# Mikubill/sketch2img

Hardware: AMD Instinct MI355X
Metric: sketch-guided images/sec whole-node, SD1.5 512px 50-step DDIM (higher is better)
Workload: dtype fp16

## Files before the change

### sketch2img_amd/csrc/attention.hip

```cpp
#include "common.h"
#include <stdlib.h>
#include <type_traits>

namespace {

struct AttnParams {
  const half_t* Q; int ldq;
  const half_t* K; int ldk;
  const half_t* V; int ldv;
  const half_t* Vt; int ldvt;
  const half_t* dO; int lddo;
  half_t* O; int ldo;
  half_t* O2; int ldo2;
  float* lse;
  const float* delta;
  const half_t* Of; int ldof;
  float* delta_out;
  int batch, heads, Nq, Nkv, kv_stride, dh;
  float scale;
  int nx;
};

struct BlkMap { int bx, h, b; };
__device__ __forceinline__ BlkMap attn_block_map(const AttnParams& p) {
// ... 630 lines not shown
    soff[j] = ok ? (unsigned)(row * (isv ? p.ldvt : p.ldk) + pc * 8) * 2u : ATT_OOB;
    sdst[j] = ok ? (isv ? vrow * VP + pc * 8 : row * KP + pc * 8) : -1;
  }
  half8_t sreg[MAXPC], sreg2[DEEP ? MAXPC : 1];
  auto stage_load_to = [&](half8_t (&r)[MAXPC], int t) {
    const unsigned sk = (unsigned)t * 64u * (unsigned)p.ldk * 2u, sv = (unsigned)t * 64u * (unsigned)p.ldvt * 2u;
#pragma unroll
    for (int j = 0; j < MAXPC; ++j) r[j] = sisv[j] ? buf_half8(rv, soff[j], sv) : buf_half8(rk, soff[j], sk);
  };
  auto stage_store_from = [&](const half8_t (&r)[MAXPC], int t) {
    half_t* const ks = lds + (t & (NK - 1)) * KSZ;
    half_t* const vs = lds + VBASE + (t & (NV - 1)) * VSZ;
#pragma unroll
    for (int j = 0; j < MAXPC; ++j)
      if (sdst[j] >= 0) st_half8((sisv[j] ? vs : ks) + sdst[j], r[j]);
  };
  auto stage_load = [&](int t) { stage_load_to(sreg, t); };
  auto stage_store = [&](int t) { stage_store_from(sreg, t); };
  for (int i = tid; i < (NK + NV) * 64; i += NTHR) {
    const int slot = i >> 6, row = i & 63;
    if (slot < NK) {
      for (int c = PK * 8; c < D16 * 16; c += 8) st_half8(lds + slot * KSZ + row * KP + c, zero_half8());
    } else {
      half_t* const vr = lds + VBASE + (slot - NK) * VSZ + row * VP;
      if (ONES) {
        const half8_t one = {(half_t)1.f, 0, 0, 0, 0, 0, 0, 0};
        st_half8(vr + PK * 8, one);
      } else {
        for (int c = PK * 8; c < ND * 16; c += 8) st_half8(vr + c, zero_half8());
      }
    }
  }
  const int nt = (p.Nkv + 63) >> 6;
  stage_load(0);
  stage_store(0);
  if (nt > 1) { stage_load(1); stage_store(1); }
  if (nt > 2) stage_load(2);

  float16_t sA[2], sB[2];
  uint4_t pA[2][2], pB[2][2];
  float4_t o[2][ND];
  float nm = 0.f, l = 0.f;
#pragma unroll
  for (int qt = 0; qt < 2; ++qt)
#pragma unroll
    for (int u = 0; u < ND; ++u) o[qt][u] = float4_t{0.f, 0.f, 0.f, 0.f};
  constexpr float REF_SLACK = 8.f;
  const int vlane = (16 * (g >> 1) + 4 * (g & 1) + (l16 >> 2)) * VP + 4 * (l16 & 3);
  const int klane = l32 * KP + 8 * hi;

  auto read_k = [&](int t, half8_t (&kf)[2][D16]) {
    const half_t* Ks = lds + (t & (NK - 1)) * KSZ + klane;
#pragma unroll
    for (int kt = 0; kt < 2; ++kt)
#pragma unroll
      for (int ks = 0; ks < D16; ++ks) kf[kt][ks] = (PROBE & 16) ? qf[ks] : ld_half8(Ks + 32 * kt * KP + 16 * ks);
  };
  auto read_v = [&](int t, half8_t (&vf)[ND][2]) {
    const half_t* Vs = lds + VBASE + (t & (NV - 1)) * VSZ + vlane;
#pragma unroll
    for (int u = 0; u < ND; ++u)
#pragma unroll
      for (int sv = 0; sv < 2; ++sv) {
        if (PROBE & 16) { vf[u][sv] = qf[(u + sv) % D16]; continue; }
        const half4_t lo = tr_read(Vs + (32 * sv) * VP + 16 * u), hh = tr_read(Vs + (32 * sv + 8) * VP + 16 * u);
        vf[u][sv] = half8_t{lo[0], lo[1], lo[2], lo[3], hh[0], hh[1], hh[2], hh[3]};
      }
  };
  auto qk = [&](const half8_t (&kf)[2][D16], float16_t (&s)[2]) {
    if (PROBE & 2) { asm volatile("" : "+v"(s[0]), "+v"(s[1])); return; }
    const float16_t init = {nm, nm, nm, nm, nm, nm, nm, nm, nm, nm, nm, nm, nm, nm, nm, nm};
#pragma unroll
    for (int ks = 0; ks < D16; ++ks)
#pragma unroll
      for (int kt = 0; kt < 2; ++kt)
        s[kt] = __builtin_amdgcn_mfma_f32_32x32x16_f16(kf[kt][ks], qf[ks], ks == 0 ? init : s[kt], 0, 0, 0);
  };
  auto pv = [&](const half8_t (&vf)[ND][2], const uint4_t (&pb)[2][2]) {
    if (PROBE & 2) return;
#pragma unroll
    for (int sv = 0; sv < 2; ++sv)
#pragma unroll
      for (int u = 0; u < ND; ++u)
#pragma unroll
        for (int qt = 0; qt < 2; ++qt)
          o[qt][u] = __builtin_amdgcn_mfma_f32_16x16x32_f16(vf[u][sv], __builtin_bit_cast(half8_t, pb[qt][sv]), o[qt][u], 0, 0, 0);
  };
  auto expo = [&](const float16_t (&s)[2], uint4_t (&pb)[2][2]) {
    float ps = 0.f;
#pragma unroll
    for (int kt = 0; kt < 2; ++kt) {
      unsigned pk[8];
#pragma unroll
      for (int j = 0; j < 8; ++j) {
        const float e0 = (PROBE & 1) ? s[kt][2 * j] : __builtin_amdgcn_exp2f(s[kt][2 * j]);
        const float e1 = (PROBE & 1) ? s[kt][2 * j + 1] : __builtin_amdgcn_exp2f(s[kt][2 * j + 1]);
        if (!ONES) ps += e0 + e1;
        const half2_t h2 = {(half_t)e0, (half_t)e1};
        pk[j] = __builtin_bit_cast(unsigned, h2);
      }
#pragma unroll
      for (int j = 0; j < 4; ++j) {
        const auto r = __builtin_amdgcn_permlane16_swap(pk[j], pk[j + 4], false, false);
        pb[0][kt][j] = r[0];
        pb[1][kt][j] = r[1];
      }
    }
    if (!ONES) l += ps;
  };
  auto tile_max = [&](auto is_last, int t, float16_t (&s)[2]) {
    const int kv0 = t * 64;
    if (decltype(is_last)::value && kv0 + 64 > p.Nkv) {
      int lim = p.Nkv - kv0 - 4 * hi;
      asm volatile("" : "+v"(lim));
#pragma unroll
      for (int kt = 0; kt < 2; ++kt)
#pragma unroll
        for (int r = 0; r < 16; ++r)
          if (32 * kt + (r & 3) + 8 * (r >> 2) >= lim) s[kt][r] = NEG_BIG;
    }
    float m8[8];
#pragma unroll
    for (int j = 0; j < 5; ++j) m8[j] = max3f(s[0][3 * j], s[0][3 * j + 1], s[0][3 * j + 2]);
    m8[5] = max3f(s[0][15], s[1][0], s[1][1]);
    m8[6] = max3f(s[1][2], s[1][3], s[1][4]);
    m8[7] = max3f(s[1][5], s[1][6], s[1][7]);
    float mx = max3f(max3f(m8[0], m8[1], m8[2]), max3f(m8[3], m8[4], m8[5]), max3f(m8[6], m8[7], s[1][8]));
    mx = max3f(mx, max3f(s[1][9], s[1][10], s[1][11]), max3f(s[1][12], s[1][13], s[1][14]));
    return max3f(mx, s[1][15], mx);
  };
  auto rebase = [&](bool first, float mx, float16_t (&s)[2]) {
    mx = max3f(mx, __shfl_xor(mx, 32, 64), mx);
    const float delta = (first || mx > REF_SLACK) ? mx : 0.f;
    const float alpha = first ? 1.f : __builtin_amdgcn_exp2f(-delta);
    nm -= delta;
    l *= alpha;
    const float aA = __shfl(alpha, l16, 64), aB = __shfl(alpha, 16 + l16, 64);
#pragma unroll
    for (int u = 0; u < ND; ++u) { o[0][u] *= aA; o[1][u] *= aB; }
#pragma unroll
    for (int kt = 0; kt < 2; ++kt) s[kt] -= delta;
  };
#ifdef SKG_PHASES
  unsigned long long att_acc[6] = {0, 0, 0, 0, 0, 0};
#endif
  auto step = [&](auto has_pv, auto has_qk, int t, float16_t (&sc)[2], float16_t (&sn)[2], uint4_t (&pp)[2][2], uint4_t (&pc)[2][2]) {
    constexpr bool HAS_PV = decltype(has_pv)::value, HAS_QK = decltype(has_qk)::value;
    ATT_T(ta);
    half8_t vf[ND][2], kf[2][D16];
    if constexpr (HAS_PV) read_v(t - 1, vf);
    if constexpr (HAS_QK) read_k(t + 1, kf);
    if constexpr (HAS_PV) pv(vf, pp);
    const float mx = tile_max(std::integral_constant<bool, !HAS_QK>{}, t, sc);
    ATT_T(tb);
    if (__builtin_amdgcn_ballot_w64(t == 0 || mx > REF_SLACK) != 0) rebase(t == 0, mx, sc);
    ATT_T(tc);
    if constexpr (HAS_QK) qk(kf, sn);
    expo(sc, pc);
    ATT_T(td);
    if (!(PROBE & 4)) {
      if (t + 2 < nt) stage_store(t + 2);
      if (t + 3 < nt) stage_load(t + 3);
    }
    asm volatile("s_waitcnt lgkmcnt(0)" ::: "memory");
    ATT_T(te);
    __builtin_amdgcn_sched_barrier(0);
    if (!(PROBE & 8)) asm volatile("s_barrier" ::: "memory");
    __builtin_amdgcn_sched_barrier(0);
    ATT_T(tf);
    ATT_ACC(0, ta, tb); ATT_ACC(1, tb, tc); ATT_ACC(2, tc, td); ATT_ACC(3, td, te); ATT_ACC(4, te, tf); ATT_ACC(5, ta, tf);
  };
  using T_ = std::true_type;
  using F_ = std::false_type;
  if constexpr (DEEP) {
    half8_t kfA[2][D16], kfB[2][D16], vfA[ND][2], vfB[ND][2];
    auto dstep = [&](auto has_pv, auto has_qk, int t, float16_t (&sc)[2], float16_t (&sn)[2], uint4_t (&pp)[2][2], uint4_t (&pc)[2][2],
                     half8_t (&kfu)[2][D16], half8_t (&kff)[2][D16], half8_t (&vfu)[ND][2], half8_t (&vff)[ND][2], half8_t (&sst)[MAXPC]) {
      constexpr bool HAS_PV = decltype(has_pv)::value, HAS_QK = decltype(has_qk)::value;
      ATT_T(ta);
      if (t + 2 < nt) read_k(t + 2, kff);
      read_v(t, vff);
      if constexpr (HAS_PV) pv(vfu, pp);
      const float mx = tile_max(std::integral_constant<bool, !HAS_QK>{}, t, sc);
      ATT_T(tb);
      if (__builtin_amdgcn_ballot_w64(t == 0 || mx > REF_SLACK) != 0) rebase(t == 0, mx, sc);
      ATT_T(tc);
      if constexpr (HAS_QK) qk(kfu, sn);
      expo(sc, pc);
      ATT_T(td);
      if (!(PROBE & 4)) {
        if (t + 3 < nt) stage_store_from(sst, t + 3);
        if (t + 5 < nt) stage_load_to(sst, t + 5);
      }
      asm volatile("s_waitcnt lgkmcnt(0)" ::: "memory");
      ATT_T(te);
      __builtin_amdgcn_sched_barrier(0);
      if (!(PROBE & 8)) asm volatile("s_barrier" ::: "memory");
      __builtin_amdgcn_sched_barrier(0);
      ATT_T(tf);
      ATT_ACC(0, ta, tb); ATT_ACC(1, tb, tc); ATT_ACC(2, tc, td); ATT_ACC(3, td, te); ATT_ACC(4, te, tf); ATT_ACC(5, ta, tf);
    };
#define DSTEP_EVEN(PV_, QK_, t_) dstep(PV_{}, QK_{}, t_, sA, sB, pB, pA, kfB, kfA, vfB, vfA, sreg2)
#define DSTEP_ODD(PV_, QK_, t_) dstep(PV_{}, QK_{}, t_, sB, sA, pA, pB, kfA, kfB, vfA, vfB, sreg)
    __syncthreads();
    read_k(0, kfA);
    qk(kfA, sA);
    if (nt > 1) read_k(1, kfB);
    asm volatile("s_waitcnt lgkmcnt(0)\n\ts_barrier" ::: "memory");
    if (nt > 2) stage_store(2);
    if (nt > 3) stage_load_to(sreg2, 3);
    if (nt > 4) stage_load_to(sreg, 4);
    asm volatile("s_waitcnt lgkmcnt(0)\n\ts_barrier" ::: "memory");
    if (nt > 1) DSTEP_EVEN(F_, T_, 0); else DSTEP_EVEN(F_, F_, 0);
    int t = 1;
    for (; t + 2 < nt; t += 2) {
      DSTEP_ODD(T_, T_, t);
      DSTEP_EVEN(T_, T_, t + 1);
    }
    if (nt > 1) {
      if (t + 1 < nt) {
        DSTEP_ODD(T_, T_, t);
        DSTEP_EVEN(T_, F_, t + 1);
        pv(vfA, pA);
      } else {
        DSTEP_ODD(T_, F_, t);
        pv(vfB, pB);
      }
    } else {
      pv(vfA, pA);
    }
#undef DSTEP_EVEN
#undef DSTEP_ODD
  } else {

  __syncthreads();
  {
    half8_t kf[2][D16];
    read_k(0, kf);
    qk(kf, sA);
  }
  asm volatile("s_waitcnt lgkmcnt(0)\n\ts_barrier" ::: "memory");
  if (nt > 1) step(F_{}, T_{}, 0, sA, sB, pB, pA); else step(F_{}, F_{}, 0, sA, sB, pB, pA);
  int t = 1;
  for (; t + 2 < nt; t += 2) {
    step(T_{}, T_{}, t, sB, sA, pA, pB);
    step(T_{}, T_{}, t + 1, sA, sB, pB, pA);
  }
  bool last_in_a = true;
  if (nt > 1) {
    if (t + 1 < nt) {
      step(T_{}, T_{}, t, sB, sA, pA, pB);
      step(T_{}, F_{}, t + 1, sA, sB, pB, pA);
    } else {
      step(T_{}, F_{}, t, sB, sA, pA, pB);
      last_in_a = false;
    }
  }
  {
    half8_t vf[ND][2];
    read_v(nt - 1, vf);
    if (last_in_a) pv(vf, pA); else pv(vf, pB);
  }

  }
#ifdef SKG_PHASES
  if (lane == 0 && blockIdx.x < (1 << 13)) {
    for (int j = 0; j < 6; ++j) g_attn_phase[blockIdx.x * NW + wave][j] = att_acc[j];
    g_attn_phase[blockIdx.x * NW + wave][6] = nt;
  }
#endif
  float liA, liB;
  if (ONES) {
    liA = __shfl(o[0][ND - 1][0], 32 + l16, 64);
    liB = __shfl(o[1][ND - 1][0], 32 + l16, 64);
  } else {
    const float ls = l + __shfl_xor(l, 32, 64);
    liA = __shfl(ls, l16, 64);
    liB = __shfl(ls, 16 + l16, 64);
  }
#pragma unroll
  for (int qt = 0; qt < 2; ++qt) {
    const int q = q0 + 16 * qt + l16;
    const float inv = 1.f / (qt ? liB : liA);
    if (q < p.Nq) {
      half_t* orow = p.O + (size_t)(b * p.Nq + q) * p.ldo + h * dh;
#pragma unroll
      for (int u = 0; u < ND; ++u) {
        const int d = 16 * u + 4 * g;
        if (d < dh) {
          const half4_t v = {(half_t)(o[qt][u][0] * inv), (half_t)(o[qt][u][1] * inv), (half_t)(o[qt][u][2] * inv), (half_t)(o[qt][u][3] * inv)};
          st_half4(orow + d, v);
        }
      }
    }
  }
  if (p.lse) {
    const float li = (lane & 16) ? liB : liA;
    if (hi == 0 && q0 + l32 < p.Nq) p.lse[((size_t)b * p.heads + h) * p.Nq + q0 + l32] = (log2f(li) - nm) * LN2;
  }
}

#endif

template <int KS, int ND, int QT>
__global__ __launch_bounds__(256, 2) void attn_bwd_dq_kernel(const AttnParams p) {
  constexpr int KP = KS * 32 + 16;
  __shared__ __attribute__((aligned(16))) half_t Ks[64 * KP];
  __shared__ __attribute__((aligned(16))) half_t Vr[64 * KP];
  const int lane = threadIdx.x & 63, wave = threadIdx.x >> 6;
  const int l16 = lane & 15, g = lane >> 4;
  const BlkMap bm = attn_block_map(p);
  const int b = bm.b, h = bm.h;
  const int dh = p.dh;
  int q[QT];
  bool qok[QT];
  half8_t qf[QT][KS], dof[QT][KS];
  float4_t nlse[QT], ndl[QT];
  float4_t dq[QT][ND];
#pragma unroll
  for (int i = 0; i < QT; ++i) {
    q[i] = bm.bx * (64 * QT) + (wave * QT + i) * 16 + l16;
    qok[i] = q[i] < p.Nq;
#pragma unroll
    for (int ks = 0; ks < KS; ++ks) {
      const int c = 32 * ks + 8 * g;
      const bool ok = qok[i] && c < dh;
      qf[i][ks] = ok ? ld_half8(p.Q + (size_t)(b * p.Nq + q[i]) * p.ldq + h * dh + c) : zero_half8();
      dof[i][ks] = ok ? ld_half8(p.dO + (size_t)(b * p.Nq + q[i]) * p.lddo + h * dh + c) : zero_half8();
    }
    const size_t sidx = ((size_t)b * p.heads + h) * p.Nq + (qok[i] ? q[i] : 0);
    float dl;
    if (p.Of) {
      float sm = 0.f;
#pragma unroll
      for (int ks = 0; ks < KS; ++ks) {
        const int c = 32 * ks + 8 * g;
        if (qok[i] && c < dh) {
          const half8_t of = ld_half8(p.Of + (size_t)(b * p.Nq + q[i]) * p.ldof + h * dh + c);
#pragma unroll
          for (int j = 0; j < 8; ++j) sm += (float)of[j] * (float)dof[i][ks][j];
        }
      }
      sm += __shfl_xor(sm, 16, 64);
      sm += __shfl_xor(sm, 32, 64);
      if (g == 0 && qok[i]) p.delta_out[sidx] = sm;
      dl = sm;
    } else {
      dl = qok[i] ? p.delta[sidx] : 0.f;
    }
    const float nl = qok[i] ? -p.lse[sidx] * LOG2E : NEG_BIG, nd = qok[i] ? -dl : 0.f;
    nlse[i] = float4_t{nl, nl, nl, nl};
    ndl[i] = float4_t{nd, nd, nd, nd};
#pragma unroll
    for (int u = 0; u < ND; ++u) dq[i][u] = float4_t{0.f, 0.f, 0.f, 0.f};
  }
  const float sc = p.scale * LOG2E;
#pragma unroll
  for (int i = 0; i < QT; ++i)
#pragma unroll
    for (int ks = 0; ks < KS; ++ks)
#pragma unroll
      for (int j = 0; j < 8; ++j) qf[i][ks][j] = (half_t)((float)qf[i][ks][j] * sc);

  const half_t* Kb = p.K + (size_t)b * p.kv_stride * p.ldk + h * dh;
  const half_t* Vb = p.V + (size_t)b * p.kv_stride * p.ldv + h * dh;
  const int nt = (p.Nkv + 63) / 64;
  RowRegs<KS> rk, rv;
  const RowSrc<KS> sk = row_src<KS>(Kb, p.ldk, p.kv_stride, dh), sv = row_src<KS>(Vb, p.ldv, p.kv_stride, dh);
  const int tlane = (4 * g + (l16 >> 2)) * KP + 4 * (l16 & 3);
  rows_load_buf<KS>(rk, sk, p.ldk, 0);
  rows_load_buf<KS>(rv, sv, p.ldv, 0);
  for (int t0 = 0; t0 < nt; ++t0) {
    const int kv0 = t0 * 64;
    __syncthreads();
    rows_store<KS>(rk, Ks);
    rows_store<KS>(rv, Vr);
    __syncthreads();
    if (t0 + 1 < nt) {
      rows_load_buf<KS>(rk, sk, p.ldk, kv0 + 64);
      rows_load_buf<KS>(rv, sv, p.ldv, kv0 + 64);
    }
    float4_t s[QT][4], dp[QT][4];
#pragma unroll
    for (int t = 0; t < 4; ++t) {
#pragma unroll
      for (int ks = 0; ks < KS; ++ks) {
        const int off = (16 * t + l16) * KP + 32 * ks + 8 * g;
        const half8_t kfr = ld_half8(Ks + off), vfr = ld_half8(Vr + off);
#pragma unroll
        for (int i = 0; i < QT; ++i) {
          s[i][t] = __builtin_amdgcn_mfma_f32_16x16x32_f16(kfr, qf[i][ks], ks == 0 ? nlse[i] : s[i][t], 0, 0, 0);
          dp[i][t] = __builtin_amdgcn_mfma_f32_16x16x32_f16(vfr, dof[i][ks], ks == 0 ? ndl[i] : dp[i][t], 0, 0, 0);
        }
      }
    }
    half8_t sb[QT][2];
#pragma unroll
    for (int i = 0; i < QT; ++i) {
      if (kv0 + 64 > p.Nkv) {
        const int lim = p.Nkv - kv0 - 4 * g;
#pragma unroll
        for (int t = 0; t < 4; ++t)
#pragma unroll
          for (int r = 0; r < 4; ++r)
            if (16 * t + r >= lim) s[i][t][r] = NEG_BIG;
      }
#pragma unroll
      for (int t = 0; t < 4; ++t)
#pragma unroll
        for (int r = 0; r < 4; ++r) s[i][t][r] = __builtin_amdgcn_exp2f(s[i][t][r]) * dp[i][t][r];
      pack_p(s[i], sb[i]);
    }
#pragma unroll
    for (int u = 0; u < ND; ++u)
#pragma unroll
      for (int k2 = 0; k2 < 2; ++k2) {
        const half8_t ktf = tfrag_rows<KP>(Ks + tlane, u, k2);
#pragma unroll
        for (int i = 0; i < QT; ++i) dq[i][u] = __builtin_amdgcn_mfma_f32_16x16x32_f16(ktf, sb[i][k2], dq[i][u], 0, 0, 0);
      }
  }
#pragma unroll
  for (int i = 0; i < QT; ++i) {
    if (!qok[i]) continue;
    half_t* orow = p.O + (size_t)(b * p.Nq + q[i]) * p.ldo + h * dh;
#pragma unroll
    for (int u = 0; u < ND; ++u) {
      const int d = 16 * u + 4 * g;
      if (d < dh) {
        half4_t v = {(half_t)(dq[i][u][0] * p.scale), (half_t)(dq[i][u][1] * p.scale), (half_t)(dq[i][u][2] * p.scale),
                     (half_t)(dq[i][u][3] * p.scale)};
        st_half4(orow + d, v);
      }
    }
  }
}

template <int KS, int ND, int KT>
__global__ __launch_bounds__(256, (KS >= 5 ? 1 : 2)) void attn_bwd_dkv_kernel(const AttnParams p) {
  constexpr int KP = KS * 32 + 16;
  __shared__ __attribute__((aligned(16))) half_t Qs[64 * KP];
  __shared__ __attribute__((aligned(16))) half_t Ds[64 * KP];
  __shared__ __attribute__((aligned(16))) float lse_s[64], del_s[64];
  const int lane = threadIdx.x & 63, wave = threadIdx.x >> 6;
  const int l16 = lane & 15, g = lane >> 4;
  const BlkMap bm = attn_block_map(p);
  const int b = bm.b, h = bm.h;
  const int dh = p.dh;
  int kv[KT];
  bool kok[KT];
  half8_t kf[KT][KS], vf[KT][KS];
#pragma unroll
  for (int i = 0; i < KT; ++i) {
    kv[i] = bm.bx * (64 * KT) + (wave * KT + i) * 16 + l16;
    kok[i] = kv[i] < p.Nkv;
#pragma unroll
    for (int ks = 0; ks < KS; ++ks) {
      const int c = 32 * ks + 8 * g;
      const bool ok = kok[i] && c < dh;
      kf[i][ks] = ok ? ld_half8(p.K + (size_t)(b * p.kv_stride + kv[i]) * p.ldk + h * dh + c) : zero_half8();
      vf[i][ks] = ok ? ld_half8(p.V + (size_t)(b * p.kv_stride + kv[i]) * p.ldv + h * dh + c) : zero_half8();
    }
  }
  const float sc = p.scale * LOG2E;
#pragma unroll
  for (int i = 0; i < KT; ++i)
#pragma unroll
    for (int ks = 0; ks < KS; ++ks)
#pragma unroll
      for (int j = 0; j < 8; ++j) kf[i][ks][j] = (half_t)((float)kf[i][ks][j] * sc);
  float4_t dk[KT][ND], dv[KT][ND];
#pragma unroll
  for (int i = 0; i < KT; ++i)
#pragma unroll
    for (int u = 0; u < ND; ++u) {
      dk[i][u] = float4_t{0.f, 0.f, 0.f, 0.f};
      dv[i][u] = float4_t{0.f, 0.f, 0.f, 0.f};
    }
  const half_t* Qb = p.Q + (size_t)b * p.Nq * p.ldq + h * dh;
  const half_t* Db = p.dO + (size_t)b * p.Nq * p.lddo + h * dh;
  const size_t sbase = ((size_t)b * p.heads + h) * p.Nq;
  const int nt = (p.Nq + 63) / 64;
  RowRegs<KS> rq, rd;
  float r_lse = 0.f, r_del = 0.f;
  const RowSrc<KS> sq = row_src<KS>(Qb, p.ldq, p.Nq, dh), sd = row_src<KS>(Db, p.lddo, p.Nq, dh);
  const int tlane = (4 * g + (l16 >> 2)) * KP + 4 * (l16 & 3);
  auto prefetch = [&](int q0) {
    rows_load_buf<KS>(rq, sq, p.ldq, q0);
    rows_load_buf<KS>(rd, sd, p.lddo, q0);
    if (threadIdx.x < 64) {
      const int qq = q0 + threadIdx.x;
      r_lse = qq < p.Nq ? -p.lse[sbase + qq] * LOG2E : NEG_BIG;
      r_del = qq < p.Nq ? -p.delta[sbase + qq] : 0.f;
    }
  };
  prefetch(0);
  for (int t0 = 0; t0 < nt; ++t0) {
    const int q0 = t0 * 64;
    __syncthreads();
    rows_store<KS>(rq, Qs);
    rows_store<KS>(rd, Ds);
    if (threadIdx.x < 64) { lse_s[threadIdx.x] = r_lse; del_s[threadIdx.x] = r_del; }
    __syncthreads();
    if (t0 + 1 < nt) prefetch(q0 + 64);
    float4_t s[KT][4], dp[KT][4];
#pragma unroll
    for (int t = 0; t < 4; ++t) {
      const float4_t nl = *reinterpret_cast<const float4_t*>(lse_s + 16 * t + 4 * g);
#pragma unroll
      for (int ks = 0; ks < KS; ++ks) {
        const int off = (16 * t + l16) * KP + 32 * ks + 8 * g;
        const half8_t qfr = ld_half8(Qs + off), dfr = ld_half8(Ds + off);
#pragma unroll
        for (int i = 0; i < KT; ++i) {
          s[i][t] = __builtin_amdgcn_mfma_f32_16x16x32_f16(qfr, kf[i][ks], ks == 0 ? nl : s[i][t], 0, 0, 0);
          dp[i][t] = __builtin_amdgcn_mfma_f32_16x16x32_f16(dfr, vf[i][ks], ks == 0 ? float4_t{0.f, 0.f, 0.f, 0.f} : dp[i][t], 0, 0, 0);
        }
      }
    }
    half8_t pb[KT][2], sb[KT][2];
#pragma unroll
    for (int i = 0; i < KT; ++i) {
      float4_t ds[4];
#pragma unroll
      for (int t = 0; t < 4; ++t)
#pragma unroll
        for (int r = 0; r < 4; ++r) {
          const float pr = __builtin_amdgcn_exp2f(s[i][t][r]);
          s[i][t][r] = pr;
          ds[t][r] = pr * (dp[i][t][r] + del_s[16 * t + 4 * g + r]);
        }
      pack_p(s[i], pb[i]);
      pack_p(ds, sb[i]);
    }
#pragma unroll
    for (int u = 0; u < ND; ++u)
#pragma unroll
      for (int k2 = 0; k2 < 2; ++k2) {
        const half8_t dtf = tfrag_rows<KP>(Ds + tlane, u, k2), qtf = tfrag_rows<KP>(Qs + tlane, u, k2);
#pragma unroll
        for (int i = 0; i < KT; ++i) {
          dv[i][u] = __builtin_amdgcn_mfma_f32_16x16x32_f16(dtf, pb[i][k2], dv[i][u], 0, 0, 0);
          dk[i][u] = __builtin_amdgcn_mfma_f32_16x16x32_f16(qtf, sb[i][k2], dk[i][u], 0, 0, 0);
        }
      }
  }
#pragma unroll
  for (int i = 0; i < KT; ++i) {
    if (!kok[i]) continue;
    half_t* krow = p.O + (size_t)(b * p.kv_stride + kv[i]) * p.ldo + h * dh;
    half_t* vrow = p.O2 + (size_t)(b * p.kv_stride + kv[i]) * p.ldo2 + h * dh;
#pragma unroll
    for (int u = 0; u < ND; ++u) {
      const int d = 16 * u + 4 * g;
      if (d < dh) {
        half4_t a = {(half_t)(dk[i][u][0] * p.scale), (half_t)(dk[i][u][1] * p.scale),
                     (half_t)(dk[i][u][2] * p.scale), (half_t)(dk[i][u][3] * p.scale)};
        half4_t c = {(half_t)dv[i][u][0], (half_t)dv[i][u][1], (half_t)dv[i][u][2], (half_t)dv[i][u][3]};
        st_half4(krow + d, a);
        st_half4(vrow + d, c);
      }
    }
  }
}

__global__ __launch_bounds__(256) void attn_delta_kernel(const half_t* __restrict__ O, int ldo,
                                                         const half_t* __restrict__ dO, int lddo,
                                                         float* __restrict__ delta, int batch, int heads, int Nq,
                                                         int dh) {
  const size_t total = (size_t)batch * Nq * heads;
  const size_t item = ((size_t)blockIdx.x * 256 + threadIdx.x) >> 4;
  const int sub = threadIdx.x & 15;
  float s = 0.f;
  if (item < total) {
    const int h = (int)(item % heads);
    const size_t row = item / heads;
    for (int c = sub * 8; c < dh; c += 128) {
      const half8_t a = ld_half8(O + row * ldo + h * dh + c);
      const half8_t d = ld_half8(dO + row * lddo + h * dh + c);
#pragma unroll
      for (int j = 0; j < 8; ++j) s += (float)a[j] * (float)d[j];
    }
  }
#pragma unroll
  for (int o = 8; o > 0; o >>= 1) s += __shfl_xor(s, o, 64);
  if (item < total && sub == 0) {
    const int h = (int)(item % heads);
    const size_t row = item / heads;
    const size_t b = row / Nq, q = row - b * Nq;
    delta[(b * heads + h) * Nq + q] = s;
  }
}

inline int attn_var();
template <int KS, int ND, bool VROW>
static void attn_fwd_launch_qt(AttnParams& p, hipStream_t st) {
  const int var = attn_var();
  const long rows = (long)p.heads * p.batch;
  if constexpr (ND == 3) {
    if (var == 9 || (var == 0 && skg_cdiv(p.Nq, 192) * rows >= 1024)) {
      p.nx = skg_cdiv(p.Nq, 192);
      hipLaunchKernelGGL((attn_fwd_kernel<KS, ND, 3, false, 2 | (3 << 2), VROW>), dim3((unsigned)(p.nx * rows)), dim3(256), 0, st, p);
      return;
    }
  } else if constexpr (VROW) {
    if (var == 8) {
      p.nx = skg_cdiv(p.Nq, 256);
      hipLaunchKernelGGL((attn_fwd_kernel<KS, ND, 4, false, 2 | (2 << 2), VROW>), dim3((unsigned)(p.nx * rows)), dim3(256), 0, st, p);
      return;
    }
  }
  p.nx = skg_cdiv(p.Nq, 128);
  const dim3 grid((unsigned)(p.nx * rows));
  if (ND == 4 && var != 7)
    hipLaunchKernelGGL((attn_fwd_kernel<KS, ND, 2, false, 2 | (3 << 2), VROW>), grid, dim3(256), 0, st, p);
  else
    hipLaunchKernelGGL((attn_fwd_kernel<KS, ND, 2, false, 0, VROW>), grid, dim3(256), 0, st, p);
}
#define SKG_ATTN_VARIANTS(KS_, ND_, grid2, VROW_) attn_fwd_launch_qt<KS_, ND_, VROW_>(p, st)

#define SKG_ATTN_FWD_DISPATCH(grid1, grid2, VROW_)                                                                 \
  switch (p.dh) {                                                                                                  \
    case 16: hipLaunchKernelGGL((attn_fwd_kernel<1, 1, 2, false, 0, VROW_>), grid2, dim3(256), 0, st, p); break;   \
    case 32: hipLaunchKernelGGL((attn_fwd_kernel<1, 2, 2, false, 0, VROW_>), grid2, dim3(256), 0, st, p); break;   \
    case 40: SKG_ATTN_VARIANTS(2, 3, grid2, VROW_); break;                                                         \
    case 64: SKG_ATTN_VARIANTS(2, 4, grid2, VROW_); break;                                                         \
    case 80: hipLaunchKernelGGL((attn_fwd_kernel<3, 5, 2, false, 0, VROW_>), grid2, dim3(256), 0, st, p); break;   \
    case 160: hipLaunchKernelGGL((attn_fwd_kernel<5, 10, 1, false, 0, VROW_>), grid1, dim3(256), 0, st, p); break; \
    default: return SKG_E_UNSUPPORTED;                                                                             \
  }

#define SKG_ATTN_FWD_CAUSAL_DISPATCH(grid2)                                                               \
  switch (p.dh) {                                                                                        \
    case 16: hipLaunchKernelGGL((attn_fwd_kernel<1, 1, 2, true>), grid2, dim3(256), 0, st, p); break;    \
    case 32: hipLaunchKernelGGL((attn_fwd_kernel<1, 2, 2, true>), grid2, dim3(256), 0, st, p); break;    \
    case 64: hipLaunchKernelGGL((attn_fwd_kernel<2, 4, 2, true>), grid2, dim3(256), 0, st, p); break;    \
    default: return SKG_E_UNSUPPORTED;                                                                   \
  }

inline int attn_var() {
  static const int v = getenv("SKG_ATTN_VAR") ? atoi(getenv("SKG_ATTN_VAR")) : 0;
  return v;
}

inline bool common_ok(int batch, int heads, int Nq, int Nkv, int kv_stride, int dh, bool kv8 = true) {
  return batch > 0 && heads > 0 && Nq > 0 && Nkv > 0 && kv_stride >= Nkv && (!kv8 || kv_stride % 8 == 0) && dh % 8 == 0;
}

}

extern "C" int skg_attn_fwd(const void* Q, int ldq, const void* K, int ldk, const void* Vt, int ldvt, void* O,
                            int ldo, float* lse, int batch, int heads, int Nq, int Nkv, int kv_stride, int dh,
                            float scale, unsigned flags, void* stream) {
  const bool causal = flags & SKG_ATTN_CAUSAL, vrow = flags & SKG_ATTN_ROWV, resident = flags & SKG_ATTN_RESIDENT_KV;
  SKG_REQUIRE(!(flags & ~(SKG_ATTN_CAUSAL | SKG_ATTN_ROWV | SKG_ATTN_RESIDENT_KV)) && !(causal && vrow) && (!resident || vrow));
  SKG_REQUIRE(Q && K && Vt && O && common_ok(batch, heads, Nq, Nkv, kv_stride, dh, !vrow));
  SKG_REQUIRE(ldq % 8 == 0 && ldk % 8 == 0 && ldvt % 8 == 0 && ldo % 4 == 0);
  SKG_REQUIRE(skg_aligned(Q, 16) && skg_aligned(K, 16) && skg_aligned(Vt, 16) && skg_aligned(O, 8));
  AttnParams p{};
  p.Q = (const half_t*)Q; p.ldq = ldq; p.K = (const half_t*)K; p.ldk = ldk; p.Vt = (const half_t*)Vt; p.ldvt = ldvt;
  p.O = (half_t*)O; p.ldo = ldo; p.lse = lse;
  p.batch = batch; p.heads = heads; p.Nq = Nq; p.Nkv = Nkv; p.kv_stride = kv_stride; p.dh = dh; p.scale = scale;
  hipStream_t st = (hipStream_t)stream;
  static const bool no_short = getenv("SKG_NO_ATTN_SHORT") != nullptr;
  if (vrow && !causal && kv_stride <= 80 && !no_short && (dh == 40 || dh == 64 || dh == 80 || dh == 160)) {
    long qch = ((long)heads * batch * Nq / 1024 + 63) / 64 * 64;
    qch = qch < 64 ? 64 : (qch > 512 ? 512 : qch);
    p.nx = skg_cdiv(Nq, (int)qch);
    dim3 gs((unsigned)p.nx * heads * batch);
    switch (dh) {
      case 40: hipLaunchKernelGGL((attn_fwd_short_kernel<2, 3>), gs, dim3(256), 0, st, p, (int)qch); break;
      case 64: hipLaunchKernelGGL((attn_fwd_short_kernel<2, 4>), gs, dim3(256), 0, st, p, (int)qch); break;
      case 80: hipLaunchKernelGGL((attn_fwd_short_kernel<3, 5>), gs, dim3(256), 0, st, p, (int)qch); break;
      default: hipLaunchKernelGGL((attn_fwd_short_kernel<5, 10>), gs, dim3(256), 0, st, p, (int)qch); break;
    }
    SKG_CHECK_LAUNCH("skg_attn_fwd (short keys)");
    return SKG_OK;
  }
  const int rtiles = kv_stride <= 160 ? 10 : 15;
  if (resident && kv_stride > 80 && kv_stride <= 240 && !no_short && (dh == 40 || dh == 64 || dh == 80 || (dh == 160 && rtiles == 10))) {
    long qch = ((long)heads * batch * Nq / 1024 + 63) / 64 * 64;
    qch = qch < 128 ? 128 : (qch > 512 ? 512 : qch);
    p.nx = skg_cdiv(Nq, (int)qch);
    dim3 gs((unsigned)p.nx * heads * batch);
    if (rtiles == 10) {
      switch (dh) {
        case 40: hipLaunchKernelGGL((attn_fwd_short_kernel<2, 3, 10>), gs, dim3(256), 0, st, p, (int)qch); break;
        case 64: hipLaunchKernelGGL((attn_fwd_short_kernel<2, 4, 10>), gs, dim3(256), 0, st, p, (int)qch); break;
        case 80: hipLaunchKernelGGL((attn_fwd_short_kernel<3, 5, 10>), gs, dim3(256), 0, st, p, (int)qch); break;
        default: hipLaunchKernelGGL((attn_fwd_short_kernel<5, 10, 10>), gs, dim3(256), 0, st, p, (int)qch); break;
      }
    } else {
      switch (dh) {
        case 40: hipLaunchKernelGGL((attn_fwd_short_kernel<2, 3, 15>), gs, dim3(256), 0, st, p, (int)qch); break;
        case 64: hipLaunchKernelGGL((attn_fwd_short_kernel<2, 4, 15>), gs, dim3(256), 0, st, p, (int)qch); break;
        default: hipLaunchKernelGGL((attn_fwd_short_kernel<3, 5, 15>), gs, dim3(256), 0, st, p, (int)qch); break;
      }
    }
    SKG_CHECK_LAUNCH("skg_attn_fwd (resident keys)");
    return SKG_OK;
  }
#if defined(SKG_LAB) || defined(SKG_PHASES)
  static const bool no8 = getenv("SKG_NO_ATTN8") != nullptr || getenv("SKG_ATTN8") == nullptr;
  static const int form8 = getenv("SKG_ATTN8") ? atoi(getenv("SKG_ATTN8")) : 0;
  if (vrow && !causal && !no8 && (dh == 40 || dh == 64) && (long)skg_cdiv(Nq, 256) * heads * batch >= 192) {
    const int qpw = form8 == 2 ? 128 : 256;
    p.nx = skg_cdiv(Nq, qpw);
    dim3 g8((unsigned)p.nx * heads * batch);
#ifdef SKG_PHASES
    static const int probe8 = getenv("SKG_ATTN8_PROBE") ? atoi(getenv("SKG_ATTN8_PROBE")) : 0;
    if (probe8 && dh == 40 && form8 == 2) {
      switch (probe8) {
        case 1: hipLaunchKernelGGL((attn_fwd8_kernel<3, 3, true, 4, 3, 1>), g8, dim3(256), 0, st, p); break;
        case 2: hipLaunchKernelGGL((attn_fwd8_kernel<3, 3, true, 4, 3, 2>), g8, dim3(256), 0, st, p); break;
        case 4: hipLaunchKernelGGL((attn_fwd8_kernel<3, 3, true, 4, 3, 4>), g8, dim3(256), 0, st, p); break;
        case 8: hipLaunchKernelGGL((attn_fwd8_kernel<3, 3, true, 4, 3, 8>), g8, dim3(256), 0, st, p); break;
        case 12: hipLaunchKernelGGL((attn_fwd8_kernel<3, 3, true, 4, 3, 12>), g8, dim3(256), 0, st, p); break;
        case 16: hipLaunchKernelGGL((attn_fwd8_kernel<3, 3, true, 4, 3, 16>), g8, dim3(256), 0, st, p); break;
        case 28: hipLaunchKernelGGL((attn_fwd8_kernel<3, 3, true, 4, 3, 28>), g8, dim3(256), 0, st, p); break;
        case 29: hipLaunchKernelGGL((attn_fwd8_kernel<3, 3, true, 4, 3, 29>), g8, dim3(256), 0, st, p); break;
        default: hipLaunchKernelGGL((attn_fwd8_kernel<3, 3, true, 4, 3, 30>), g8, dim3(256), 0, st, p); break;
      }
      SKG_CHECK_LAUNCH("skg_attn_fwd (8 waves, probe)");
      return SKG_OK;
    }
#endif
    if (form8 == 2) {
      if (dh == 40) hipLaunchKernelGGL((attn_fwd8_kernel<3, 3, true, 4, 3>), g8, dim3(256), 0, st, p);
      else hipLaunchKernelGGL((attn_fwd8_kernel<4, 4, false, 4, 2>), g8, dim3(256), 0, st, p);
    } else {
      if (dh == 40) hipLaunchKernelGGL((attn_fwd8_kernel<3, 3, true>), g8, dim3(512), 0, st, p);
      else hipLaunchKernelGGL((attn_fwd8_kernel<4, 4, false>), g8, dim3(512), 0, st, p);
    }
    SKG_CHECK_LAUNCH("skg_attn_fwd (8 waves)");
    return SKG_OK;
  }
#endif
  p.nx = skg_cdiv(Nq, dh == 160 ? 64 : 128);
  dim3 grid((unsigned)p.nx * heads * batch);
  if (causal) {
    SKG_REQUIRE(dh != 160 && !vrow);
    SKG_ATTN_FWD_CAUSAL_DISPATCH(grid);
  } else if (vrow) {
    SKG_ATTN_FWD_DISPATCH(grid, grid, true);
  } else {
    SKG_ATTN_FWD_DISPATCH(grid, grid, false);
  }
  SKG_CHECK_LAUNCH("skg_attn_fwd");
  return SKG_OK;
}

extern "C" int skg_attn_bwd_delta(const void* O, int ldo, const void* dO, int lddo, float* delta, int batch,
                                  int heads, int Nq, int dh, void* stream) {
  SKG_REQUIRE(O && dO && delta && batch > 0 && heads > 0 && Nq > 0 && dh % 8 == 0 && ldo % 8 == 0 && lddo % 8 == 0);
  SKG_REQUIRE(skg_aligned(O, 16) && skg_aligned(dO, 16));
  const size_t total = (size_t)batch * Nq * heads;
  hipLaunchKernelGGL(attn_delta_kernel, dim3((unsigned)((total * 16 + 255) / 256)), dim3(256), 0,
                     (hipStream_t)stream, (const half_t*)O, ldo, (const half_t*)dO, lddo, delta, batch, heads, Nq, dh);
  SKG_CHECK_LAUNCH("skg_attn_bwd_delta");
  return SKG_OK;
}

extern "C" int skg_attn_bwd_dq(const void* Q, int ldq, const void* K, int ldk, const void* V, int ldv, const void* dO, int lddo,
                               const void* O, int ldo, const float* lse, const float* delta, float* delta_out, void* dQ, int lddq,
                               int batch, int heads, int Nq, int Nkv, int kv_stride, int dh, float scale, void* stream) {
  if (delta) { O = nullptr; ldo = 0; delta_out = nullptr; }
  SKG_REQUIRE(Q && K && V && dO && lse && (delta || (O && delta_out)) && dQ && common_ok(batch, heads, Nq, Nkv, kv_stride, dh, false));
  SKG_REQUIRE(!O || (ldo % 8 == 0 && skg_aligned(O, 16)));
  SKG_REQUIRE(ldq % 8 == 0 && ldk % 8 == 0 && ldv % 8 == 0 && lddo % 8 == 0 && lddq % 4 == 0);
  SKG_REQUIRE(skg_aligned(Q, 16) && skg_aligned(K, 16) && skg_aligned(V, 16) && skg_aligned(dO, 16) && skg_aligned(dQ, 8));
  AttnParams p{};
  p.Q = (const half_t*)Q; p.ldq = ldq; p.K = (const half_t*)K; p.ldk = ldk; p.V = (const half_t*)V; p.ldv = ldv;
  p.dO = (const half_t*)dO; p.lddo = lddo;
  p.lse = const_cast<float*>(lse); p.delta = delta; p.O = (half_t*)dQ; p.ldo = lddq;
  p.Of = (const half_t*)O; p.ldof = ldo; p.delta_out = delta_out;
  p.batch = batch; p.heads = heads; p.Nq = Nq; p.Nkv = Nkv; p.kv_stride = kv_stride; p.dh = dh; p.scale = scale;
  hipStream_t st = (hipStream_t)stream;
  p.nx = skg_cdiv(Nq, dh <= 40 ? 128 : 64);
  dim3 grid((unsigned)p.nx * heads * batch);
  switch (dh) {
    case 16: hipLaunchKernelGGL((attn_bwd_dq_kernel<1, 1, 2>), grid, dim3(256), 0, st, p); break;
    case 32: hipLaunchKernelGGL((attn_bwd_dq_kernel<1, 2, 2>), grid, dim3(256), 0, st, p); break;
    case 40: hipLaunchKernelGGL((attn_bwd_dq_kernel<2, 3, 2>), grid, dim3(256), 0, st, p); break;
    case 64: hipLaunchKernelGGL((attn_bwd_dq_kernel<2, 4, 1>), grid, dim3(256), 0, st, p); break;
    case 80: hipLaunchKernelGGL((attn_bwd_dq_kernel<3, 5, 1>), grid, dim3(256), 0, st, p); break;
    case 160: hipLaunchKernelGGL((attn_bwd_dq_kernel<5, 10, 1>), grid, dim3(256), 0, st, p); break;
    default: return SKG_E_UNSUPPORTED;
  }
  SKG_CHECK_LAUNCH("skg_attn_bwd_dq");
  return SKG_OK;
}

extern "C" int skg_attn_bwd_dkv(const void* Q, int ldq, const void* K, int ldk,
                                const void* V, int ldv, const void* dO, int lddo,
                                const float* lse, const float* delta, void* dK, int lddk, void* dV, int lddv,
                                int batch, int heads, int Nq, int Nkv, int kv_stride, int dh, float scale, void* stream) {
  SKG_REQUIRE(Q && K && V && dO && lse && delta && dK && dV && common_ok(batch, heads, Nq, Nkv, kv_stride, dh, false));
  SKG_REQUIRE(ldq % 8 == 0 && ldk % 8 == 0 && ldv % 8 == 0 && lddo % 8 == 0 && lddk % 4 == 0 && lddv % 4 == 0);
  SKG_REQUIRE(skg_aligned(Q, 16) && skg_aligned(K, 16) && skg_aligned(V, 16) &&
              skg_aligned(dO, 16) && skg_aligned(dK, 8) && skg_aligned(dV, 8));
  AttnParams p{};
  p.Q = (const half_t*)Q; p.ldq = ldq; p.K = (const half_t*)K; p.ldk = ldk;
  p.V = (const half_t*)V; p.ldv = ldv; p.dO = (const half_t*)dO; p.lddo = lddo;
  p.lse = const_cast<float*>(lse); p.delta = delta; p.O = (half_t*)dK; p.ldo = lddk;
  p.O2 = (half_t*)dV; p.ldo2 = lddv;
  p.batch = batch; p.heads = heads; p.Nq = Nq; p.Nkv = Nkv; p.kv_stride = kv_stride; p.dh = dh; p.scale = scale;
  hipStream_t st = (hipStream_t)stream;
  p.nx = skg_cdiv(Nkv, dh <= 40 ? 128 : 64);
  dim3 grid((unsigned)p.nx * heads * batch);
  switch (dh) {
    case 16: hipLaunchKernelGGL((attn_bwd_dkv_kernel<1, 1, 2>), grid, dim3(256), 0, st, p); break;
    case 32: hipLaunchKernelGGL((attn_bwd_dkv_kernel<1, 2, 2>), grid, dim3(256), 0, st, p); break;
    case 40: hipLaunchKernelGGL((attn_bwd_dkv_kernel<2, 3, 2>), grid, dim3(256), 0, st, p); break;
    case 64: hipLaunchKernelGGL((attn_bwd_dkv_kernel<2, 4, 1>), grid, dim3(256), 0, st, p); break;
    case 80: hipLaunchKernelGGL((attn_bwd_dkv_kernel<3, 5, 1>), grid, dim3(256), 0, st, p); break;
    case 160: hipLaunchKernelGGL((attn_bwd_dkv_kernel<5, 10, 1>), grid, dim3(256), 0, st, p); break;
    default: return SKG_E_UNSUPPORTED;
  }
  SKG_CHECK_LAUNCH("skg_attn_bwd_dkv");
  return SKG_OK;
}

#ifdef SKG_PHASES
extern "C" int skg_debug_attn_phases(void* host_out, int nwaves) {
  return (int)hipMemcpyFromSymbol(host_out, HIP_SYMBOL(g_attn_phase), (size_t)nwaves * 8 * sizeof(unsigned long long));
}
#endif
```

Baseline: 6.057.

## Double-buffer LDS and split tiles into halves in attention backward kernels

Attention backward dq and dkv kernels gain template parameters for splitting each 64-row tile into halves, optional double-buffered shared memory stages, and per-head-dim waves-per-EU launch bounds. Double buffering removes one barrier per tile and overlaps staging the next tile with compute. Half-tile processing shrinks live score registers to allow higher occupancy. For the dkv half-split path, delta is folded into the MFMA accumulator init. The risks are more LDS per block and possible register spills at the higher occupancy targets.

```diff
diff --git a/sketch2img_amd/csrc/attention.hip b/sketch2img_amd/csrc/attention.hip
--- a/sketch2img_amd/csrc/attention.hip
+++ b/sketch2img_amd/csrc/attention.hip
@@ -956,11 +956,19 @@
 
 #endif
 
-template <int KS, int ND, int QT>
-__global__ __launch_bounds__(256, 2) void attn_bwd_dq_kernel(const AttnParams p) {
+template <int TPH>
+__device__ __forceinline__ void pack_block(const float4_t (&s)[TPH], half8_t (&pb)[TPH / 2]) {
+#pragma unroll
+  for (int kk = 0; kk < TPH / 2; ++kk)
+#pragma unroll
+    for (int i = 0; i < 8; ++i) pb[kk][i] = (half_t)s[2 * kk + (i >> 2)][i & 3];
+}
+
+template <int KS, int ND, int QT, int NH, int ST, int WV>
+__global__ __launch_bounds__(256, WV) void attn_bwd_dq_kernel(const AttnParams p) {
   constexpr int KP = KS * 32 + 16;
-  __shared__ __attribute__((aligned(16))) half_t Ks[64 * KP];
-  __shared__ __attribute__((aligned(16))) half_t Vr[64 * KP];
+  constexpr int TSZ = 64 * KP;
+  __shared__ __attribute__((aligned(16))) half_t lds[ST * 2 * TSZ];
   const int lane = threadIdx.x & 63, wave = threadIdx.x >> 6;
   const int l16 = lane & 15, g = lane >> 4;
   const BlkMap bm = attn_block_map(p);
@@ -1022,57 +1030,89 @@
   RowRegs<KS> rk, rv;
   const RowSrc<KS> sk = row_src<KS>(Kb, p.ldk, p.kv_stride, dh), sv = row_src<KS>(Vb, p.ldv, p.kv_stride, dh);
   const int tlane = (4 * g + (l16 >> 2)) * KP + 4 * (l16 & 3);
+  auto tile = [&](const half_t* __restrict__ Ks, int kv0) {
+    const half_t* __restrict__ Vr = Ks + TSZ;
+    constexpr int TPH = 4 / NH, FPH = 2 / NH;
+#pragma unroll
+    for (int hb = 0; hb < NH; ++hb) {
+      float4_t s[QT][TPH], dp[QT][TPH];
+#pragma unroll
+      for (int tt = 0; tt < TPH; ++tt) {
+        const int t = hb * TPH + tt;
+#pragma unroll
+        for (int ks = 0; ks < KS; ++ks) {
+          const int off = (16 * t + l16) * KP + 32 * ks + 8 * g;
+          const half8_t kfr = ld_half8(Ks + off), vfr = ld_half8(Vr + off);
+#pragma unroll
+          for (int i = 0; i < QT; ++i) {
+            s[i][tt] = __builtin_amdgcn_mfma_f32_16x16x32_f16(kfr, qf[i][ks], ks == 0 ? nlse[i] : s[i][tt], 0, 0, 0);
+            dp[i][tt] = __builtin_amdgcn_mfma_f32_16x16x32_f16(vfr, dof[i][ks], ks == 0 ? ndl[i] : dp[i][tt], 0, 0, 0);
+          }
+        }
+      }
+      half8_t sb[QT][FPH];
+#pragma unroll
+      for (int i = 0; i < QT; ++i) {
+        if (kv0 + 64 > p.Nkv) {
+          const int lim = p.Nkv - kv0 - 4 * g;
+#pragma unroll
+          for (int tt = 0; tt < TPH; ++tt)
+#pragma unroll
+            for (int r = 0; r < 4; ++r)
+              if (16 * (hb * TPH + tt) + r >= lim) s[i][tt][r] = NEG_BIG;
+        }
+#pragma unroll
+        for (int tt = 0; tt < TPH; ++tt)
+#pragma unroll
+          for (int r = 0; r < 4; ++r) s[i][tt][r] = __builtin_amdgcn_exp2f(s[i][tt][r]) * dp[i][tt][r];
+        pack_block<TPH>(s[i], sb[i]);
+      }
+#pragma unroll
+      for (int u = 0; u < ND; ++u)
+#pragma unroll
+        for (int kk = 0; kk < FPH; ++kk) {
+          const half8_t ktf = tfrag_rows<KP>(Ks + tlane, u, hb * FPH + kk);
+#pragma unroll
+          for (int i = 0; i < QT; ++i) dq[i][u] = __builtin_amdgcn_mfma_f32_16x16x32_f16(ktf, sb[i][kk], dq[i][u], 0, 0, 0);
+        }
+    }
+  };
   rows_load_buf<KS>(rk, sk, p.ldk, 0);
   rows_load_buf<KS>(rv, sv, p.ldv, 0);
-  for (int t0 = 0; t0 < nt; ++t0) {
-    const int kv0 = t0 * 64;
+  if constexpr (ST == 1) {
+    for (int t0 = 0; t0 < nt; ++t0) {
+      const int kv0 = t0 * 64;
+      __syncthreads();
+      rows_store<KS>(rk, lds);
+      rows_store<KS>(rv, lds + TSZ);
+      __syncthreads();
+      if (t0 + 1 < nt) {
+        rows_load_buf<KS>(rk, sk, p.ldk, kv0 + 64);
+        rows_load_buf<KS>(rv, sv, p.ldv, kv0 + 64);
+      }
+      tile(lds, kv0);
+    }
+  } else {
+    rows_store<KS>(rk, lds);
+    rows_store<KS>(rv, lds + TSZ);
+    if (nt > 1) {
+      rows_load_buf<KS>(rk, sk, p.ldk, 64);
+      rows_load_buf<KS>(rv, sv, p.ldv, 64);
+    }
     __syncthreads();
-    rows_store<KS>(rk, Ks);
-    rows_store<KS>(rv, Vr);
-    __syncthreads();
-    if (t0 + 1 < nt) {
-      rows_load_buf<KS>(rk, sk, p.ldk, kv0 + 64);
-      rows_load_buf<KS>(rv, sv, p.ldv, kv0 + 64);
-    }
-    float4_t s[QT][4], dp[QT][4];
-#pragma unroll
-    for (int t = 0; t < 4; ++t) {
-#pragma unroll
-      for (int ks = 0; ks < KS; ++ks) {
-        const int off = (16 * t + l16) * KP + 32 * ks + 8 * g;
-        const half8_t kfr = ld_half8(Ks + off), vfr = ld_half8(Vr + off);
-#pragma unroll
-        for (int i = 0; i < QT; ++i) {
-          s[i][t] = __builtin_amdgcn_mfma_f32_16x16x32_f16(kfr, qf[i][ks], ks == 0 ? nlse[i] : s[i][t], 0, 0, 0);
-          dp[i][t] = __builtin_amdgcn_mfma_f32_16x16x32_f16(vfr, dof[i][ks], ks == 0 ? ndl[i] : dp[i][t], 0, 0, 0);
-        }
-      }
-    }
-    half8_t sb[QT][2];
-#pragma unroll
-    for (int i = 0; i < QT; ++i) {
-      if (kv0 + 64 > p.Nkv) {
-        const int lim = p.Nkv - kv0 - 4 * g;
-#pragma unroll
-        for (int t = 0; t < 4; ++t)
-#pragma unroll
-          for (int r = 0; r < 4; ++r)
-            if (16 * t + r >= lim) s[i][t][r] = NEG_BIG;
-      }
-#pragma unroll
-      for (int t = 0; t < 4; ++t)
-#pragma unroll
-        for (int r = 0; r < 4; ++r) s[i][t][r] = __builtin_amdgcn_exp2f(s[i][t][r]) * dp[i][t][r];
-      pack_p(s[i], sb[i]);
-    }
-#pragma unroll
-    for (int u = 0; u < ND; ++u)
-#pragma unroll
-      for (int k2 = 0; k2 < 2; ++k2) {
-        const half8_t ktf = tfrag_rows<KP>(Ks + tlane, u, k2);
-#pragma unroll
-        for (int i = 0; i < QT; ++i) dq[i][u] = __builtin_amdgcn_mfma_f32_16x16x32_f16(ktf, sb[i][k2], dq[i][u], 0, 0, 0);
-      }
+    for (int t0 = 0; t0 < nt; ++t0) {
+      tile(lds + (t0 & 1) * (2 * TSZ), t0 * 64);
+      if (t0 + 1 < nt) {
+        half_t* nxt = lds + ((t0 + 1) & 1) * (2 * TSZ);
+        rows_store<KS>(rk, nxt);
+        rows_store<KS>(rv, nxt + TSZ);
+      }
+      if (t0 + 2 < nt) {
+        rows_load_buf<KS>(rk, sk, p.ldk, (t0 + 2) * 64);
+        rows_load_buf<KS>(rv, sv, p.ldv, (t0 + 2) * 64);
+      }
+      __syncthreads();
+    }
   }
 #pragma unroll
   for (int i = 0; i < QT; ++i) {
@@ -1090,12 +1130,12 @@
   }
 }
 
-template <int KS, int ND, int KT>
-__global__ __launch_bounds__(256, (KS >= 5 ? 1 : 2)) void attn_bwd_dkv_kernel(const AttnParams p) {
+template <int KS, int ND, int KT, int NH, int ST, int WV>
+__global__ __launch_bounds__(256, WV) void attn_bwd_dkv_kernel(const AttnParams p) {
   constexpr int KP = KS * 32 + 16;
-  __shared__ __attribute__((aligned(16))) half_t Qs[64 * KP];
-  __shared__ __attribute__((aligned(16))) half_t Ds[64 * KP];
-  __shared__ __attribute__((aligned(16))) float lse_s[64], del_s[64];
+  constexpr int TSZ = 64 * KP;
+  __shared__ __attribute__((aligned(16))) half_t lds[ST * 2 * TSZ];
+  __shared__ __attribute__((aligned(16))) float stat[ST * 128];
   const int lane = threadIdx.x & 63, wave = threadIdx.x >> 6;
   const int l16 = lane & 15, g = lane >> 4;
   const BlkMap bm = attn_block_map(p);
@@ -1148,56 +1188,83 @@
       r_del = qq < p.Nq ? -p.delta[sbase + qq] : 0.f;
     }
   };
+  auto stage_store = [&](int st) {
+    rows_store<KS>(rq, lds + st * (2 * TSZ));
+    rows_store<KS>(rd, lds + st * (2 * TSZ) + TSZ);
+    if (threadIdx.x < 64) { stat[st * 128 + threadIdx.x] = r_lse; stat[st * 128 + 64 + threadIdx.x] = r_del; }
+  };
+  auto tile = [&](int st) {
+    const half_t* __restrict__ Qs = lds + st * (2 * TSZ);
+    const half_t* __restrict__ Ds = Qs + TSZ;
+    const float* __restrict__ lse_s = stat + st * 128;
+    const float* __restrict__ del_s = lse_s + 64;
+    constexpr int TPH = 4 / NH, FPH = 2 / NH;
+    constexpr bool DELC = NH == 2;
+#pragma unroll
+    for (int hb = 0; hb < NH; ++hb) {
+      float4_t s[KT][TPH], dp[KT][TPH];
+#pragma unroll
+      for (int tt = 0; tt < TPH; ++tt) {
+        const int t = hb * TPH + tt;
+        const float4_t nl = *reinterpret_cast<const float4_t*>(lse_s + 16 * t + 4 * g);
+        const float4_t nd = DELC ? *reinterpret_cast<const float4_t*>(del_s + 16 * t + 4 * g) : float4_t{0.f, 0.f, 0.f, 0.f};
+#pragma unroll
+        for (int ks = 0; ks < KS; ++ks) {
+          const int off = (16 * t + l16) * KP + 32 * ks + 8 * g;
+          const half8_t qfr = ld_half8(Qs + off), dfr = ld_half8(Ds + off);
+#pragma unroll
+          for (int i = 0; i < KT; ++i) {
+            s[i][tt] = __builtin_amdgcn_mfma_f32_16x16x32_f16(qfr, kf[i][ks], ks == 0 ? nl : s[i][tt], 0, 0, 0);
+            dp[i][tt] = __builtin_amdgcn_mfma_f32_16x16x32_f16(dfr, vf[i][ks], ks == 0 ? nd : dp[i][tt], 0, 0, 0);
+          }
+        }
+      }
+      half8_t pb[KT][FPH], sb[KT][FPH];
+#pragma unroll
+      for (int i = 0; i < KT; ++i) {
+#pragma unroll
+        for (int tt = 0; tt < TPH; ++tt)
+#pragma unroll
+          for (int r = 0; r < 4; ++r) {
+            const float pr = __builtin_amdgcn_exp2f(s[i][tt][r]);
+            s[i][tt][r] = pr;
+            dp[i][tt][r] = DELC ? pr * dp[i][tt][r] : pr * (dp[i][tt][r] + del_s[16 * (hb * TPH + tt) + 4 * g + r]);
+          }
+        pack_block<TPH>(s[i], pb[i]);
+        pack_block<TPH>(dp[i], sb[i]);
+      }
+#pragma unroll
+      for (int u = 0; u < ND; ++u)
+#pragma unroll
+        for (int kk = 0; kk < FPH; ++kk) {
+          const half8_t dtf = tfrag_rows<KP>(Ds + tlane, u, hb * FPH + kk), qtf = tfrag_rows<KP>(Qs + tlane, u, hb * FPH + kk);
+#pragma unroll
+          for (int i = 0; i < KT; ++i) {
+            dv[i][u] = __builtin_amdgcn_mfma_f32_16x16x32_f16(dtf, pb[i][kk], dv[i][u], 0, 0, 0);
+            dk[i][u] = __builtin_amdgcn_mfma_f32_16x16x32_f16(qtf, sb[i][kk], dk[i][u], 0, 0, 0);
+          }
+        }
+    }
+  };
   prefetch(0);
-  for (int t0 = 0; t0 < nt; ++t0) {
-    const int q0 = t0 * 64;
+  if constexpr (ST == 1) {
+    for (int t0 = 0; t0 < nt; ++t0) {
+      __syncthreads();
+      stage_store(0);
+      __syncthreads();
+      if (t0 + 1 < nt) prefetch(t0 * 64 + 64);
+      tile(0);
+    }
+  } else {
+    stage_store(0);
+    if (nt > 1) prefetch(64);
     __syncthreads();
-    rows_store<KS>(rq, Qs);
-    rows_store<KS>(rd, Ds);
-    if (threadIdx.x < 64) { lse_s[threadIdx.x] = r_lse; del_s[threadIdx.x] = r_del; }
-    __syncthreads();
-    if (t0 + 1 < nt) prefetch(q0 + 64);
-    float4_t s[KT][4], dp[KT][4];
-#pragma unroll
-    for (int t = 0; t < 4; ++t) {
-      const float4_t nl = *reinterpret_cast<const float4_t*>(lse_s + 16 * t + 4 * g);
-#pragma unroll
-      for (int ks = 0; ks < KS; ++ks) {
-        const int off = (16 * t + l16) * KP + 32 * ks + 8 * g;
-        const half8_t qfr = ld_half8(Qs + off), dfr = ld_half8(Ds + off);
-#pragma unroll
-        for (int i = 0; i < KT; ++i) {
-          s[i][t] = __builtin_amdgcn_mfma_f32_16x16x32_f16(qfr, kf[i][ks], ks == 0 ? nl : s[i][t], 0, 0, 0);
-          dp[i][t] = __builtin_amdgcn_mfma_f32_16x16x32_f16(dfr, vf[i][ks], ks == 0 ? float4_t{0.f, 0.f, 0.f, 0.f} : dp[i][t], 0, 0, 0);
-        }
-      }
-    }
-    half8_t pb[KT][2], sb[KT][2];
-#pragma unroll
-    for (int i = 0; i < KT; ++i) {
-      float4_t ds[4];
-#pragma unroll
-      for (int t = 0; t < 4; ++t)
-#pragma unroll
-        for (int r = 0; r < 4; ++r) {
-          const float pr = __builtin_amdgcn_exp2f(s[i][t][r]);
-          s[i][t][r] = pr;
-          ds[t][r] = pr * (dp[i][t][r] + del_s[16 * t + 4 * g + r]);
-        }
-      pack_p(s[i], pb[i]);
-      pack_p(ds, sb[i]);
-    }
-#pragma unroll
-    for (int u = 0; u < ND; ++u)
-#pragma unroll
-      for (int k2 = 0; k2 < 2; ++k2) {
-        const half8_t dtf = tfrag_rows<KP>(Ds + tlane, u, k2), qtf = tfrag_rows<KP>(Qs + tlane, u, k2);
-#pragma unroll
-        for (int i = 0; i < KT; ++i) {
-          dv[i][u] = __builtin_amdgcn_mfma_f32_16x16x32_f16(dtf, pb[i][k2], dv[i][u], 0, 0, 0);
-          dk[i][u] = __builtin_amdgcn_mfma_f32_16x16x32_f16(qtf, sb[i][k2], dk[i][u], 0, 0, 0);
-        }
-      }
+    for (int t0 = 0; t0 < nt; ++t0) {
+      tile(t0 & 1);
+      if (t0 + 1 < nt) stage_store((t0 + 1) & 1);
+      if (t0 + 2 < nt) prefetch((t0 + 2) * 64);
+      __syncthreads();
+    }
   }
 #pragma unroll
   for (int i = 0; i < KT; ++i) {
@@ -1433,12 +1500,12 @@
   p.nx = skg_cdiv(Nq, dh <= 40 ? 128 : 64);
   dim3 grid((unsigned)p.nx * heads * batch);
   switch (dh) {
-    case 16: hipLaunchKernelGGL((attn_bwd_dq_kernel<1, 1, 2>), grid, dim3(256), 0, st, p); break;
-    case 32: hipLaunchKernelGGL((attn_bwd_dq_kernel<1, 2, 2>), grid, dim3(256), 0, st, p); break;
-    case 40: hipLaunchKernelGGL((attn_bwd_dq_kernel<2, 3, 2>), grid, dim3(256), 0, st, p); break;
-    case 64: hipLaunchKernelGGL((attn_bwd_dq_kernel<2, 4, 1>), grid, dim3(256), 0, st, p); break;
-    case 80: hipLaunchKernelGGL((attn_bwd_dq_kernel<3, 5, 1>), grid, dim3(256), 0, st, p); break;
-    case 160: hipLaunchKernelGGL((attn_bwd_dq_kernel<5, 10, 1>), grid, dim3(256), 0, st, p); break;
+    case 16: hipLaunchKernelGGL((attn_bwd_dq_kernel<1, 1, 2, 1, 1, 2>), grid, dim3(256), 0, st, p); break;
+    case 32: hipLaunchKernelGGL((attn_bwd_dq_kernel<1, 2, 2, 1, 1, 2>), grid, dim3(256), 0, st, p); break;
+    case 40: hipLaunchKernelGGL((attn_bwd_dq_kernel<2, 3, 2, 2, 2, 3>), grid, dim3(256), 0, st, p); break;
+    case 64: hipLaunchKernelGGL((attn_bwd_dq_kernel<2, 4, 1, 2, 2, 3>), grid, dim3(256), 0, st, p); break;
+    case 80: hipLaunchKernelGGL((attn_bwd_dq_kernel<3, 5, 1, 2, 1, 4>), grid, dim3(256), 0, st, p); break;
+    case 160: hipLaunchKernelGGL((attn_bwd_dq_kernel<5, 10, 1, 1, 1, 2>), grid, dim3(256), 0, st, p); break;
     default: return SKG_E_UNSUPPORTED;
   }
   SKG_CHECK_LAUNCH("skg_attn_bwd_dq");
@@ -1463,12 +1530,12 @@
   p.nx = skg_cdiv(Nkv, dh <= 40 ? 128 : 64);
   dim3 grid((unsigned)p.nx * heads * batch);
   switch (dh) {
-    case 16: hipLaunchKernelGGL((attn_bwd_dkv_kernel<1, 1, 2>), grid, dim3(256), 0, st, p); break;
-    case 32: hipLaunchKernelGGL((attn_bwd_dkv_kernel<1, 2, 2>), grid, dim3(256), 0, st, p); break;
-    case 40: hipLaunchKernelGGL((attn_bwd_dkv_kernel<2, 3, 2>), grid, dim3(256), 0, st, p); break;
-    case 64: hipLaunchKernelGGL((attn_bwd_dkv_kernel<2, 4, 1>), grid, dim3(256), 0, st, p); break;
-    case 80: hipLaunchKernelGGL((attn_bwd_dkv_kernel<3, 5, 1>), grid, dim3(256), 0, st, p); break;
-    case 160: hipLaunchKernelGGL((attn_bwd_dkv_kernel<5, 10, 1>), grid, dim3(256), 0, st, p); break;
+    case 16: hipLaunchKernelGGL((attn_bwd_dkv_kernel<1, 1, 2, 1, 1, 2>), grid, dim3(256), 0, st, p); break;
+    case 32: hipLaunchKernelGGL((attn_bwd_dkv_kernel<1, 2, 2, 1, 1, 2>), grid, dim3(256), 0, st, p); break;
+    case 40: hipLaunchKernelGGL((attn_bwd_dkv_kernel<2, 3, 2, 2, 2, 3>), grid, dim3(256), 0, st, p); break;
+    case 64: hipLaunchKernelGGL((attn_bwd_dkv_kernel<2, 4, 1, 1, 1, 2>), grid, dim3(256), 0, st, p); break;
+    case 80: hipLaunchKernelGGL((attn_bwd_dkv_kernel<3, 5, 1, 2, 1, 3>), grid, dim3(256), 0, st, p); break;
+    case 160: hipLaunchKernelGGL((attn_bwd_dkv_kernel<5, 10, 1, 2, 1, 1>), grid, dim3(256), 0, st, p); break;
     default: return SKG_E_UNSUPPORTED;
   }
   SKG_CHECK_LAUNCH("skg_attn_bwd_dkv");
```

Result: no change. 6.089, median of 6 (+0.5%).
